# RaffaeleGalliera/melissa

Hardware: AMD Instinct MI355X
Metric: env-steps/s (agent-decisions/s) L-DGN 50-node (higher is better)
Workload: dtype f32 (f32a)

## Files before the change

include/melissa_hip.h:

```cpp
#ifndef MELISSA_HIP_H
#define MELISSA_HIP_H

#include <stddef.h>
#include <stdint.h>

#ifdef __cplusplus
extern "C" {
#endif

typedef int32_t mel_status;
#define MEL_OK                 0
#define MEL_ERR_INVALID_ARG   -1
#define MEL_ERR_SHAPE         -2
#define MEL_ERR_UNSUPPORTED   -3
#define MEL_ERR_WORKSPACE     -4
#define MEL_ERR_LAUNCH        -5

#define MEL_MAX_NODES        128
#define MEL_SET_WORDS(n)     (((n) + 63) / 64)
#define MEL_NODE_COLS          8
#define MEL_MAX_HEAD_LAYERS    6

#define MEL_MODEL_LDGN         0
#define MEL_MODEL_HLDGN        1
// ... 30 lines not shown
    int32_t n_layers;
} mel_mlp;

typedef struct mel_weights {
    int32_t model;
    int32_t in_dim;
    int32_t n_actions;
    int32_t dueling;
    mel_mlp   encoder;
    mel_gatv2 conv1;
    mel_gatv2 conv2;
    mel_mlp   q_head;
    mel_mlp   v_head;
    int32_t precision;
    int32_t flags;
    const void* prepared;
    const void* tables;
    int32_t tables_nodes;
    int32_t reserved;
} mel_weights;
#define MEL_FWD_PLAN_READY 1
#define MEL_FWD_INTEGER_FEATURES 2

#define MEL_PREC_F32  0
#define MEL_PREC_BF16 1
#define MEL_PREC_F32_SPLIT 2
#define MEL_PREC_F32_AUTO 3

size_t mel_prepared_weights_bytes(const mel_weights* w);
mel_status mel_prepare_weights(const mel_weights* w, void* prepared, size_t bytes, void* stream);

size_t mel_feature_tables_bytes(const mel_weights* w, int32_t n_nodes);
mel_status mel_prepare_feature_tables(const mel_weights* w, int32_t n_nodes, void* tables, size_t bytes, void* stream);

size_t mel_workspace_bytes(const mel_weights* w, int64_t bs, int32_t n_nodes);

mel_status mel_ldgn_forward(const mel_weights* w, const float* obs, int64_t bs, int32_t n_nodes,
                            int32_t obs_width, float* logits, void* workspace, size_t ws_bytes,
                            void* stream);

typedef struct mel_select {
    int32_t*        act;
    float           eps;
    uint32_t        seed;
    const uint32_t* step_dev;
    const uint64_t* live;
    int32_t         n_nodes;
    int32_t         reserved;
    const float*    eps_dev;
} mel_select;

size_t mel_workspace_bytes_agents(const mel_weights* w, int64_t bs, int32_t n_nodes, int64_t rows_cap);
mel_status mel_plan_pointers(const mel_weights* w, int64_t bs, int32_t n_nodes, int64_t rows_cap, void* workspace,
                             void** out5);
mel_status mel_ldgn_forward_agents(const mel_weights* w, const float* obs, int64_t bs, int32_t n_nodes,
                                   int32_t obs_stride, const uint64_t* agent_mask, int64_t rows_cap,
                                   float* logits, int32_t* row_offsets, const mel_select* select,
                                   void* workspace, size_t ws_bytes, void* stream);

mel_status mel_dgnr_forward(const mel_weights* w, const float* obs, int64_t bs, int32_t n_nodes,
                            int32_t obs_width, float* logits, void* workspace, size_t ws_bytes,
                            void* stream);
mel_status mel_dgnr_forward_agents(const mel_weights* w, const float* obs, int64_t bs, int32_t n_nodes,
                                   int32_t obs_stride, const uint64_t* agent_mask, int64_t rows_cap,
                                   float* logits, int32_t* row_offsets, const mel_select* select,
                                   void* workspace, size_t ws_bytes, void* stream);
// ... 346 lines not shown
```

melissa_amd/_lib.py:

```python
from __future__ import annotations

import ctypes as C
import os

from . import build as _build

MAX_HEAD_LAYERS = 6
TD_GROUP_ROWS, TD_MAX_BATCH, TD_MAX_ACTIONS = 64, 65536, 8
MAX_NODES = 128


def set_words(n: int) -> int:
    return (int(n) + 63) // 64


def check_n_nodes(n: int, what: str):
    if not (1 <= int(n) <= MAX_NODES):
        raise ValueError(f"{what}: {n} nodes per graph is outside [1, {MAX_NODES}] - the MI355X kernels hold one graph per "
                         f"wavefront (at most two nodes per lane, node sets of at most two 64-bit words)")
MODEL_LDGN, MODEL_HLDGN, MODEL_DGNR = 0, 1, 2
CONV_GATV2, CONV_TRANSFORMER = 0, 1
AGG = {"max": 0, "mean": 1, "add": 2}
OK, ERR_INVALID_ARG, ERR_SHAPE, ERR_UNSUPPORTED, ERR_WORKSPACE, ERR_LAUNCH = 0, -1, -2, -3, -4, -5
ENV_SCALARS, ENV_LOGGER_STATS = 16, 10
S_ORIGIN, S_SELECTION, S_SKIP, S_NUM_MOVES, S_WORLD_MSGS, S_NEW_ROUND, S_EPISODE, S_MOVE_CURSOR, \
    S_DECISIONS, S_DONE_COUNT, S_EPISODES_DONE, S_ERROR, S_EP_CURSOR = range(13)
SET_HAS_MESSAGE, SET_ORIGIN, SET_INTERESTED, SET_SCRIPTED, SET_TRUNCATED, SET_ALIVE, SET_TERMINATED, \
    SET_AGENTS = range(8)

EXPORTS = ("mel_wait_counter", "mel_feature_tables_bytes", "mel_prepare_feature_tables", "mel_prepared_weights_bytes", "mel_prepare_weights", "mel_transpose_f32", "mel_episode_refill", "mel_episode_test_seeds", "mel_abi_sizeof", "mel_radius_graph", "mel_gat_forward", "mel_gat_backward", "mel_pool_forward", "mel_pool_backward",
           "mel_gemm_bf16", "mel_convert_bf16", "mel_hldgn_forward_envs", "mel_hldgn_forward_envs_select", "mel_plan_pointers", "mel_select_action_envs", "mel_dgnr_forward", "mel_dgnr_forward_agents", "mel_gemm_f32", "mel_gemm_f32_t", "mel_gemm_f32_splitk", "mel_gemm_f32_split", "mel_replay_sample", "mel_replay_sample_prio", "mel_replay_update_priority", "mel_adam_step", "mel_workspace_bytes", "mel_workspace_bytes_agents", "mel_ldgn_forward_agents",
           "mel_select_action_rows", "mel_ldgn_forward", "mel_hldgn_forward", "mel_forward_tap",
           "mel_select_action", "mel_env_state_bytes", "mel_env_bind", "mel_env_reset", "mel_env_step",
           "mel_env_observe", "mel_env_round", "mel_prof_create", "mel_prof_destroy", "mel_prof_attach", "mel_prof_reset",
           "mel_prof_read", "mel_last_error", "mel_version", "mel_mpr_sets", "mel_exploration_schedule", "mel_td_target", "mel_td_loss")
PREC_F32, PREC_BF16, PREC_F32_SPLIT, PREC_F32_AUTO = 0, 1, 2, 3
FWD_PLAN_READY = 1
FWD_INTEGER_FEATURES = 2
HEURISTICS = {None: 0, "simple_broadcast": 1, "broadcast_if_any_interested": 2, "silent": 3, "mpr": 4}
LOGGER_KEYS = ("total_messages_transmitted", "coverage", "messages_sent", "messages_received", "n_neighbours",
               "interested_agents", "coverage_interested_fraction", "coverage_interested_count",
               "uninterested_with_message", "episode_rewards_sum")
N_STAGES = 14
STAGE_NAMES = ("plan", "encoder", "conv1_lin", "conv1_lin_r", "conv1_att", "conv2_lin", "conv2_lin_r", "conv2_att",
               "head_hidden", "head_tail", "select", "env_step", "env_reset", "env_observe")


class MelLinear(C.Structure):
    _fields_ = [("weight", C.c_void_p), ("bias", C.c_void_p), ("in_dim", C.c_int32), ("out_dim", C.c_int32)]


class MelGatv2(C.Structure):
    _fields_ = [("lin_l", MelLinear), ("lin_r", MelLinear), ("att", C.c_void_p), ("bias", C.c_void_p),
                ("heads", C.c_int32), ("channels", C.c_int32), ("lin_v", MelLinear), ("kind", C.c_int32),
                ("reserved", C.c_int32)]


class MelMlp(C.Structure):
    _fields_ = [("layer", MelLinear * MAX_HEAD_LAYERS), ("n_layers", C.c_int32)]


class MelWeights(C.Structure):
    _fields_ = [("model", C.c_int32), ("in_dim", C.c_int32), ("n_actions", C.c_int32), ("dueling", C.c_int32),
# ... 163 lines not shown
    lib.mel_select_action.argtypes = [vp, vp, i64, i32, C.c_float, vp, vp, vp, vp, vp]
    lib.mel_env_state_bytes.restype = sz
    lib.mel_env_state_bytes.argtypes = [i32, i32]
    lib.mel_env_bind.restype = i32
    lib.mel_env_bind.argtypes = [E, i32, i32, vp]
    lib.mel_env_reset.restype = i32
    lib.mel_env_reset.argtypes = [E, P, vp, vp, i64, i32, O, vp]
    lib.mel_env_step.restype = i32
    lib.mel_env_step.argtypes = [E, P, vp, vp, i64, O, vp, i32, vp]
    lib.mel_env_round.restype = i32
    lib.mel_env_round.argtypes = [E, P, vp, vp, vp, vp, i32, i32, vp, C.POINTER(MelRoundReplay), vp]
    lib.mel_adam_step.restype = i32
    lib.mel_adam_step.argtypes = [C.POINTER(MelAdamTensors), C.c_float, C.c_float, C.c_float, C.c_float, C.c_float, C.c_double, vp]
    lib.mel_td_target.restype = i32
    lib.mel_td_target.argtypes = [vp, vp, vp, vp, i64, i32, vp, vp]
    lib.mel_td_loss.restype = i32
    lib.mel_td_loss.argtypes = [vp, vp, vp, vp, vp, i64, i32, i32, i32, vp, vp, vp, vp, sz, vp]
    lib.mel_replay_sample.restype = i32
    lib.mel_replay_sample.argtypes = [C.POINTER(MelRoundReplay), i64, i32, i32, i32, C.POINTER(C.c_float), C.c_uint64, vp, vp,
                                      C.POINTER(MelReplayBatch), vp]
    lib.mel_replay_sample_prio.restype = i32
    lib.mel_replay_sample_prio.argtypes = [C.POINTER(MelRoundReplay), C.POINTER(MelReplayPriority), i64, i32, i32, i32,
                                           C.POINTER(C.c_float), C.c_uint64, vp, C.POINTER(MelReplayBatch), vp, vp]
    lib.mel_replay_update_priority.restype = i32
    lib.mel_replay_update_priority.argtypes = [C.POINTER(MelReplayPriority), i64, i32, i32, i32, vp, vp, vp, vp, vp]
    lib.mel_env_observe.restype = i32
    lib.mel_env_observe.argtypes = [E, vp, i64, O, vp]
    lib.mel_mpr_sets.restype = i32
    lib.mel_mpr_sets.argtypes = [vp, i32, i32, vp, vp]
    lib.mel_feature_tables_bytes.restype = sz
    lib.mel_feature_tables_bytes.argtypes = [W, i32]
    lib.mel_prepare_feature_tables.restype = i32
    lib.mel_prepare_feature_tables.argtypes = [W, i32, vp, sz, vp]
    lib.mel_prepared_weights_bytes.restype = sz
    lib.mel_prepared_weights_bytes.argtypes = [W]
    lib.mel_prepare_weights.restype = i32
    lib.mel_prepare_weights.argtypes = [W, vp, sz, vp]
    lib.mel_transpose_f32.restype = i32
    lib.mel_transpose_f32.argtypes = [vp, i32, i64, i32, vp, i32, vp]
    lib.mel_gemm_f32.restype = i32
    lib.mel_gemm_f32.argtypes = [vp, i32, vp, vp, vp, i32, i64, i32, i32, i32, i32, vp]
    lib.mel_wait_counter.restype = i32
    lib.mel_wait_counter.argtypes = [vp, C.c_uint32, C.c_uint32, vp]
    lib.mel_episode_test_seeds.restype = i32
    lib.mel_episode_test_seeds.argtypes = [vp, i32, vp]
    lib.mel_episode_refill.restype = i32
    lib.mel_episode_refill.argtypes = [C.POINTER(MelEpisodeStream), C.POINTER(MelGraphPool), P, E, i32, i32, vp]
    lib.mel_prof_create.restype = vp
    lib.mel_prof_create.argtypes = [i32]
    lib.mel_prof_destroy.restype = None
    lib.mel_prof_destroy.argtypes = [vp]
    lib.mel_prof_attach.restype = None
    lib.mel_prof_attach.argtypes = [vp]
    lib.mel_prof_reset.restype = None
    lib.mel_prof_reset.argtypes = [vp]
    lib.mel_prof_read.restype = i32
    lib.mel_prof_read.argtypes = [vp, C.POINTER(C.c_double), C.POINTER(C.c_int64)]
    _lib = lib
    return lib


def last_error() -> str:
    return load().mel_last_error().decode()


def check(status: int, what: str = ""):
# ... 12 lines not shown
```

melissa_amd/build.py:

```python
from __future__ import annotations

import hashlib
import os
import subprocess
import sys

HERE = os.path.dirname(os.path.abspath(__file__))
CSRC = os.path.join(HERE, "csrc")
LIB_DIR = os.path.join(HERE, "lib")
LIB_PATH = os.path.join(LIB_DIR, "libmelissa_hip.so")
SOURCES = ["fwd.hip", "env.hip", "grad.hip"]
HEADERS = ["common.hpp", "gemm_f32.hpp", "gemm_walk.hpp", "gemm_bf16.hpp", "gemm_split.hpp", "gemm_ring.hpp", "gemm_launch.hpp", "plan.hpp", "plan_masks.hpp", "attention.hpp", "heads.hpp", "episode_stream.hpp", "replay_prio.hpp", "td.hpp", os.path.join("..", "..", "include", "melissa_hip.h")]


def _hipcc() -> str:
    for cand in (os.environ.get("HIPCC"), "/opt/rocm/bin/hipcc"):
        if cand and os.path.exists(cand):
            return cand
    return "hipcc"


HASH_PATH = LIB_PATH + ".srchash"


def source_hash() -> str:
    h = hashlib.sha256()
    h.update(os.environ.get("MEL_HIPCC_FLAGS", "").encode())
    for rel in SOURCES + HEADERS:
        path = os.path.join(CSRC, rel)
        if os.path.exists(path):
            h.update(rel.encode())
            h.update(open(path, "rb").read())
    return h.hexdigest()


def is_stale() -> bool:
    if not os.path.exists(LIB_PATH) or not os.path.exists(HASH_PATH):
        return True
    return open(HASH_PATH).read().strip() != source_hash()


def build_library(force: bool = False, verbose: bool = False) -> str:
    srcs = [os.path.join(CSRC, s) for s in SOURCES if os.path.exists(os.path.join(CSRC, s))]
    if not force and not is_stale():
        return LIB_PATH
# ... 22 lines not shown
```

melissa_amd/csrc/fwd.hip:

```cpp
#include <cmath>

#include "common.hpp"
#include "gemm_launch.hpp"
#include "plan.hpp"
#include "attention.hpp"
#include "heads.hpp"

namespace mel {

static thread_local char g_err[512] = "";
void set_error(const char* fmt, ...) {
    va_list ap;
    va_start(ap, fmt);
    vsnprintf(g_err, sizeof(g_err), fmt, ap);
    va_end(ap);
}

static thread_local Profiler* g_prof = nullptr;
Profiler* current_profiler() { return g_prof; }

template <int W>
__global__ __launch_bounds__(256, 2) void plan_enc_kernel(PlanListsArgs pa, GemmBatch batch, int gemm_blocks) {
    if ((int)blockIdx.x < gemm_blocks) gemm_f32_tile<2, 2, 1, 1, GEMM_MODE_ENC>(batch, (int)blockIdx.x);
    else plan_lists_body<W>(pa, (int)blockIdx.x - gemm_blocks);
}

__global__ __launch_bounds__(256, 2) void fid_enc_kernel(const float* __restrict__ obs, int bs, int n, int obs_stride, int node_cols,
                                                         PlanBuffers p, int table_rows, GemmBatch batch, int gemm_blocks) {
    if ((int)blockIdx.x < gemm_blocks) gemm_f32_tile<2, 2, 1, 1, GEMM_MODE_ENC>(batch, (int)blockIdx.x);
    else feature_ids_body(obs, bs, n, obs_stride, node_cols, p, table_rows, (int)blockIdx.x - gemm_blocks);
}

struct Dims {
    int64_t bs;
    int n;
    int64_t rows_cap;
    int64_t u1_cap;
    int64_t u2_cap;
};

static Dims make_dims(int64_t bs, int n, int64_t rows_cap, bool single_agent) {
    Dims d;
    d.bs = bs, d.n = n, d.rows_cap = rows_cap;
    d.u1_cap = single_agent ? bs * (n < 34 ? n : 34) : bs * n;
    d.u2_cap = bs * n;
    return d;
}

struct FwdLayout {
    PlanBuffers plan;
    float* h0;
    float* xl1;
    float* xr1;
    float* h1;
    float* xl2;
    float* xr2;
    float* xcat;
// ... 341 lines not shown
        }
        const bool out16 = bf && !(i + 2 == nl);
        in_q = out, ld_q = ld_v = ldo;
        in_v = out16 ? reinterpret_cast<const float*>(reinterpret_cast<const uint16_t*>(out) + q.out_dim) : out + q.out_dim;
    }
    if (bf && nl < 2) return fail(MEL_ERR_UNSUPPORTED, "bf16 path needs at least one hidden layer in the heads");
    const mel_linear& ql = w->q_head.layer[nl - 1];
    const mel_linear& vl = w->v_head.layer[nl - 1];
    StageScope t(MEL_STAGE_HEAD_TAIL, s);
    MEL_LAUNCH(dueling_tail_kernel, dim3((rows + 3) / 4), dim3(256), 0, s, in_q, ld_q, ql.in_dim, in_v, ld_v,
                       vl.in_dim, ql, vl, (int)rows, rows_dev, w->dueling, logits, select ? *select : mel_select{});
    return check_launch("dueling tail");
}

struct FeatureTables {
    float* h0;
    float* xl;
    float* xr;
};
static size_t table_elem_bytes(const mel_weights* w) { return w->precision == MEL_PREC_BF16 ? 2 : 4; }
static FeatureTables carve_tables(const mel_weights* w, int n, void* buf, size_t* bytes) {
    const size_t T = (size_t)n * FEATURE_TUPLES_PER_DEGREE, es = table_elem_bytes(w);
    const int hidden = w->encoder.layer[1].out_dim, hc = w->conv1.heads * w->conv1.channels;
    const bool hl = w->model == MEL_MODEL_HLDGN;
    const int srcw = hl ? 2 * hc : (w->conv1.kind == MEL_CONV_TRANSFORMER ? 2 * hc : hc);
    Carver c(buf);
    FeatureTables t;
    t.h0 = reinterpret_cast<float*>(c.take<char>(T * hidden * es));
    t.xl = reinterpret_cast<float*>(c.take<char>(T * srcw * es));
    t.xr = hl ? nullptr : reinterpret_cast<float*>(c.take<char>(T * hc * es));
    if (bytes) *bytes = c.off;
    return t;
}
static mel_status run_feature_tables(const mel_weights* w, const ProjWeights& pw, int n, const FeatureTables& t, hipStream_t s,
                                     bool encoder_done = false) {
    const int T = n * FEATURE_TUPLES_PER_DEGREE;
    const int hidden = w->encoder.layer[1].out_dim, hc = w->conv1.heads * w->conv1.channels;
    const int bf = w->precision == MEL_PREC_BF16, sp = w->precision == MEL_PREC_F32_SPLIT;
    const bool tconv = w->conv1.kind == MEL_CONV_TRANSFORMER, hl = w->model == MEL_MODEL_HLDGN;
    if (!encoder_done) {
        GemmArgs g;
        g.feat_domain = 1, g.in_dim = w->in_dim, g.enc_w = w->encoder.layer[0].weight, g.enc_b = w->encoder.layer[0].bias;
        g.W = pw.enc1, g.bias = w->encoder.layer[1].bias, g.bf16 = bf, g.split = sp;
        if (bf) g.W = w->encoder.layer[1].weight, g.bf16 = 0, g.y_bf16 = 1;
        g.Y = t.h0, g.ldy = hidden, g.M = T, g.N = hidden, g.K = w->encoder.layer[0].out_dim, g.relu = 1;
        StageScope sc(MEL_STAGE_ENCODER, s);
        if (mel_status st = launch_gemm(g, GEMM_MODE_ENC, s, "encoder (feature tuples)", T)) return st;
    }
    StageScope sc(MEL_STAGE_CONV1_LIN, s);
    if (hl) {
        GemmArgs g;
        g.A = t.h0, g.lda = hidden, g.W = pw.c1l, g.W_hi = pw.c1r, g.bf16 = bf, g.split = sp;
        g.bias = w->conv1.lin_l.bias, g.bias_hi = w->conv1.lin_r.bias, g.split_n = hc;
        g.Y = t.xl, g.ldy = 2 * hc, g.M = T, g.N = 2 * hc, g.K = hidden;
        return launch_gemm(g, GEMM_MODE_PLAIN, s, "conv1.lin_l|lin_r (feature tuples)");
    }
    const int srcw = tconv ? 2 * hc : hc;
    GemmArgs g[2];
    g[0].bf16 = g[1].bf16 = bf, g[0].split = g[1].split = sp;
    g[0].A = t.h0, g[0].lda = hidden, g[0].W = pw.c1l, g[0].bias = w->conv1.lin_l.bias;
    g[0].Y = t.xl, g[0].ldy = srcw, g[0].M = T, g[0].N = srcw, g[0].K = hidden;
    if (tconv) g[0].W_hi = pw.c1v, g[0].bias_hi = w->conv1.lin_v.bias, g[0].split_n = hc;
    g[1].A = t.h0, g[1].lda = hidden, g[1].W = pw.c1r, g[1].bias = w->conv1.lin_r.bias;
    g[1].Y = t.xr, g[1].ldy = hc, g[1].M = T, g[1].N = hc, g[1].K = hidden;
    const long hints[2] = {T, T};
    return launch_gemm_group(g, hints, 2, s, "conv1.lin_l + lin_r (feature tuples)", 1);
}

static mel_status ldgn_forward_impl(const mel_weights* w, const float* obs, const Dims& d, int obs_stride,
                                    const uint64_t* agent_mask, float* logits, int32_t* row_offsets_out,
                                    const mel_select* select, void* workspace, size_t ws_bytes, hipStream_t s) {
    if (!obs || !logits || !workspace) return fail(MEL_ERR_INVALID_ARG, "null obs/logits/workspace");
    const FwdLayout L = carve(w, d, workspace);
    if (ws_bytes < L.bytes) return fail(MEL_ERR_WORKSPACE, "workspace %zu < %zu bytes", ws_bytes, L.bytes);
    clear_stale_error();
    const int64_t bs = d.bs;
    const int n = d.n;
    const int node_cols = w->in_dim + 3;
    const int hidden = w->encoder.layer[1].out_dim, hc = w->conv1.heads * w->conv1.channels;
    const int latent = hidden + 2 * hc;
    const bool tconv = w->conv1.kind == MEL_CONV_TRANSFORMER;
    const int srcw = tconv ? 2 * hc : hc;
    const int R = (int)d.rows_cap, U1 = (int)d.u1_cap, U2 = (int)d.u2_cap;
    const int32_t* nL = L.plan.offL + bs;
    const int32_t* n1 = L.plan.off1 + bs;
    const int32_t* n2 = L.plan.off2 + bs;
    const bool single = agent_mask == nullptr;
    const int bf = w->precision == MEL_PREC_BF16;
    const int sp = w->precision == MEL_PREC_F32_SPLIT;
    ProjWeights pw, pw_alt;
    if (mel_status st = resolve_projections(w, L, pw, pw_alt, s)) return st;
    const long hintL = single ? bs : (n < 10 ? bs : bs * (long)(36 + n) / 18);
    const long hint1 = single ? bs * (long)(n < 8 ? n : 2 + n / 8) : (n < 10 ? bs * (long)n : bs * 2L * (18 + n) / 13);
    const long hint2 = single ? bs * (long)(n < 8 ? n : 1 + n / 4) : (n < 10 ? bs * (long)n : bs * 3L * (8 + n) / 11);
    const int T = n * FEATURE_TUPLES_PER_DEGREE;
    const bool table = (w->flags & MEL_FWD_INTEGER_FEATURES) && w->in_dim == 5 && hint1 + hint2 >= 2L * T;
    bool fused_enc = false;
    GemmArgs c2[2];
    c2[0].bf16 = c2[1].bf16 = bf, c2[0].split = c2[1].split = sp;
    c2[0].A = L.h1, c2[0].lda = hc;
    c2[0].W = pw.c2l, c2[0].bias = w->conv2.lin_l.bias;
    c2[0].Y = L.xl2, c2[0].ldy = srcw, c2[0].M = U1, c2[0].M_dev = n1, c2[0].N = srcw, c2[0].K = hc;
    if (tconv) c2[0].W_hi = pw.c2v, c2[0].bias_hi = w->conv2.lin_v.bias, c2[0].split_n = hc;
    c2[1].A = L.h1, c2[1].lda = hc, c2[1].arow = L.plan.arow_g;
    c2[1].W = pw.c2r, c2[1].bias = w->conv2.lin_r.bias;
    if (pw.alt) c2[0].Ws = pw.alt->c2l, c2[0].Ws_hi = tconv ? pw.alt->c2v : nullptr, c2[1].Ws = pw.alt->c2r;
    c2[1].Y = L.xr2, c2[1].ldy = hc, c2[1].M = R, c2[1].M_dev = nL, c2[1].N = hc, c2[1].K = hc;
    const long c2_hints[2] = {hint1, hintL};
    const ProjWeights* planes = sp ? &pw : pw.alt;
    GemmRequest c2_rq;
    c2_rq.group = true;
    PlaneBlocks c2_blocks[2];
    if (planes && hc % 4 == 0 && hc / 64 >= 4) {
        c2_blocks[0] = {planes->c2l_blk, tconv ? planes->c2v_blk : nullptr}, c2_blocks[1] = {planes->c2r_blk, nullptr};
        c2_rq.blocks = c2_blocks;
    }
    const GemmPlan conv2 = plan_gemm(c2, c2_hints, 2, c2_rq);

    {
        StageScope t(MEL_STAGE_PLAN, s);
        if (w->flags & MEL_FWD_PLAN_READY) {
            if (!agent_mask) return fail(MEL_ERR_INVALID_ARG, "MEL_FWD_PLAN_READY needs the agent-set entry points");
        } else {
            if (n > 64) MEL_LAUNCH(plan_masks_kernel<2>, dim3((bs + 3) / 4), dim3(256), 0, s, obs, (int)bs, n, obs_stride, node_cols, agent_mask, L.plan, 1);
            else MEL_LAUNCH(plan_masks_kernel<1>, dim3((bs + 3) / 4), dim3(256), 0, s, obs, (int)bs, n, obs_stride, node_cols, agent_mask, L.plan, 1);
            if (mel_status st = check_launch("plan_masks")) return st;
        }
        const int inline_scan = bs <= 8192;
        if (!inline_scan) {
            MEL_LAUNCH(plan_scan_kernel, dim3(1), dim3(1024), 0, s, (int)bs, L.plan);
            if (mel_status st = check_launch("plan_scan")) return st;
        }
        fused_enc = table && !sp && !(w->tables && w->tables_nodes == n);
        const PlanListsArgs pa{obs, (int)bs, n, obs_stride, node_cols, L.plan, row_offsets_out, tconv ? 0 : 1, inline_scan, table ? T : 0};
        if (fused_enc) {
            GemmArgs g;
            g.feat_domain = 1, g.in_dim = w->in_dim, g.enc_w = w->encoder.layer[0].weight, g.enc_b = w->encoder.layer[0].bias;
            g.W = bf ? w->encoder.layer[1].weight : pw.enc1, g.bias = w->encoder.layer[1].bias, g.y_bf16 = bf;
            g.Y = L.h0, g.ldy = hidden, g.M = T, g.N = hidden, g.K = w->encoder.layer[0].out_dim, g.relu = 1;
            GemmRequest rq;
            rq.mode = GEMM_MODE_ENC, rq.force_tile = MEL_TILE_64;
            const GemmPlan enc = plan_gemm(&g, nullptr, 1, rq);
            if (enc.status) return fail(enc.status, "encoder (feature tuples): %s", enc.why);
            const int tiles = enc.grid;
            if (n > 64) MEL_LAUNCH(plan_enc_kernel<2>, dim3(tiles + (int)((bs + 3) / 4)), dim3(256), 0, s, pa, enc.batch, tiles);
            else MEL_LAUNCH(plan_enc_kernel<1>, dim3(tiles + (int)((bs + 3) / 4)), dim3(256), 0, s, pa, enc.batch, tiles);
        } else if (n > 64) {
            MEL_LAUNCH(plan_lists_kernel<2>, dim3((bs + 3) / 4), dim3(256), 0, s, pa);
        } else {
            MEL_LAUNCH(plan_lists_kernel<1>, dim3((bs + 3) / 4), dim3(256), 0, s, pa);
        }
        if (mel_status st = check_launch("plan_lists")) return st;
    }
    {
        GemmArgs g;
        g.obs = obs, g.obs_width = obs_stride, g.n_nodes = n, g.in_dim = w->in_dim, g.node_cols = node_cols;
        g.nid = L.plan.nid2, g.enc_w = w->encoder.layer[0].weight, g.enc_b = w->encoder.layer[0].bias;
        g.W = pw.enc1, g.bias = w->encoder.layer[1].bias, g.bf16 = bf, g.split = sp;
        g.Y = L.h0, g.ldy = hidden, g.M = U2, g.M_dev = n2, g.N = hidden;
        g.K = w->encoder.layer[0].out_dim, g.relu = 1;
        StageScope t(MEL_STAGE_ENCODER, s);
        if (!table)
            if (mel_status st = launch_gemm(g, GEMM_MODE_ENC, s, "encoder", hint2)) return st;
    }
    FeatureTables ft{L.h0, L.xl1, L.xr1};
    if (table) {
        if (w->tables && w->tables_nodes == n) ft = carve_tables(w, n, const_cast<void*>(w->tables), nullptr);
        else if (mel_status st = run_feature_tables(w, pw, n, ft, s, fused_enc)) return st;
    }
    {
        GemmArgs g[2];
        g[0].bf16 = g[1].bf16 = bf, g[0].split = g[1].split = sp;
        g[0].A = L.h0, g[0].lda = hidden, g[0].W = pw.c1l, g[0].bias = w->conv1.lin_l.bias;
        g[0].Y = L.xl1, g[0].ldy = srcw, g[0].M = U2, g[0].M_dev = n2, g[0].N = srcw, g[0].K = hidden;
        if (tconv)
            g[0].W_hi = pw.c1v, g[0].bias_hi = w->conv1.lin_v.bias, g[0].split_n = hc;
        g[1].A = L.h0, g[1].lda = hidden, g[1].arow = L.plan.arow1;
        g[1].W = pw.c1r, g[1].bias = w->conv1.lin_r.bias;
        g[1].Y = L.xr1, g[1].ldy = hc, g[1].M = U1, g[1].M_dev = n1, g[1].N = hc, g[1].K = hidden;
        const long hints[2] = {hint2, hint1};
        StageScope t(MEL_STAGE_CONV1_LIN, s);
        if (!table)
            if (mel_status st = launch_gemm_group(g, hints, 2, s, "conv1.lin_l + lin_r", 1)) return st;
    }
    {
        AttArgs a{};
        a.xl = ft.xl, a.ld_l = srcw, a.xr = ft.xr, a.ld_r = hc, a.att = w->conv1.att, a.bias = w->conv1.bias;
        a.kind = w->conv1.kind, a.score_scale = 1.0f / sqrtf((float)w->conv1.channels), a.bf16 = bf;
        a.adj = L.plan.adj, a.bs = (int)bs, a.n = n;
        a.desc = L.plan.desc1, a.rows_dev = n1, a.rows_cap = U1, a.rows_hint = hint1;
        a.lanes_per_head = w->conv1.channels / (hc / 64);
        a.out = L.h1, a.ldo = hc, a.xcat = L.xcat, a.ld_cat = latent, a.hidden = hidden, a.h0 = ft.h0;
        if (conv2.kernel == GemmKernel::PLANES) a.out_planes = reinterpret_cast<uint16_t*>(L.h1);
        a.out_scale = L.plan.dm1;
        a.fid = table ? L.plan.fid : nullptr;
        StageScope t(MEL_STAGE_CONV1_ATT, s);
        if (mel_status st = launch_attend<ATT_ROWS>(a, hc, s, "conv1 attention")) return st;
    }
    {
        StageScope t(MEL_STAGE_CONV2_LIN, s);
// ... 14 lines not shown
}

}

using namespace mel;

extern "C" {

const char* mel_last_error(void) { return g_err; }
void mel_debug_fin_prof(unsigned long long* out5) {
#ifdef MEL_FIN_PROF
    (void)hipMemcpyFromSymbol(out5, HIP_SYMBOL(g_fin_prof), 5 * sizeof(unsigned long long));
    unsigned long long z[5] = {};
    (void)hipMemcpyToSymbol(HIP_SYMBOL(g_fin_prof), z, sizeof(z));
#else
    for (int i = 0; i < 5; ++i) out5[i] = 0;
#endif
}

#ifdef MEL_RING_PROF
void mel_debug_ring_prof(unsigned long long* out8) {
    (void)hipDeviceSynchronize();
    (void)hipMemcpyFromSymbol(out8, HIP_SYMBOL(g_ring_prof), 8 * sizeof(unsigned long long));
    unsigned long long z[8] = {0};
    (void)hipMemcpyToSymbol(HIP_SYMBOL(g_ring_prof), z, sizeof(z));
}
#endif
#ifdef MEL_GEMM_PROF
void mel_debug_gemm_prof(unsigned long long* out8) {
    (void)hipDeviceSynchronize();
    (void)hipMemcpyFromSymbol(out8, HIP_SYMBOL(g_gemm_prof), 8 * sizeof(unsigned long long));
    unsigned long long z[8] = {0};
    (void)hipMemcpyToSymbol(HIP_SYMBOL(g_gemm_prof), z, sizeof(z));
}
#endif
#ifdef MEL_SPLIT_PROF
void mel_debug_split_prof(unsigned long long* out16) {
    (void)hipDeviceSynchronize();
    (void)hipMemcpyFromSymbol(out16, HIP_SYMBOL(g_split_prof), 16 * sizeof(unsigned long long));
    unsigned long long z[16] = {0};
    (void)hipMemcpyToSymbol(HIP_SYMBOL(g_split_prof), z, sizeof(z));
}
#endif
#ifdef MEL_ATT_PROF
void mel_debug_att_prof(unsigned long long* out8) {
    (void)hipDeviceSynchronize();
    (void)hipMemcpyFromSymbol(out8, HIP_SYMBOL(g_att_prof), 8 * sizeof(unsigned long long));
    unsigned long long z[8] = {0};
    (void)hipMemcpyToSymbol(HIP_SYMBOL(g_att_prof), z, sizeof(z));
}
#endif
size_t mel_abi_sizeof(int32_t which) {
    switch (which) {
        case 0: return sizeof(mel_linear);
        case 1: return sizeof(mel_gatv2);
        case 2: return sizeof(mel_mlp);
        case 3: return sizeof(mel_weights);
        case 4: return sizeof(mel_select);
        case 5: return sizeof(mel_env_batch);
        case 6: return sizeof(mel_episode_pool);
        case 7: return sizeof(mel_env_obs);
        case 8: return sizeof(mel_round_replay);
        case 9: return sizeof(mel_graph_pool);
        case 10: return sizeof(mel_episode_stream);
        case 11: return sizeof(mel_replay_batch);
        case 12: return sizeof(mel_adam_tensors);
        case 13: return sizeof(mel_replay_priority);
        default: return 0;
    }
}
const char* mel_version(void) { return "melissa_hip 0.6 (gfx950)"; }

size_t mel_prepared_weights_bytes(const mel_weights* w) {
    if (!w || w->precision < MEL_PREC_F32 || w->precision > MEL_PREC_F32_AUTO) return 0;
    return prepared_elems(w) * sizeof(uint16_t);
}

size_t mel_feature_tables_bytes(const mel_weights* w, int32_t n_nodes) {
    if (!w || n_nodes < 1 || n_nodes > MEL_MAX_NODES || w->in_dim != 5 || w->encoder.n_layers != 2) return 0;
    size_t bytes = 0;
    (void)carve_tables(w, n_nodes, nullptr, &bytes);
    return bytes;
}

mel_status mel_prepare_feature_tables(const mel_weights* w, int32_t n_nodes, void* tables, size_t bytes, void* stream) {
    if (mel_status st = validate(w, w ? w->model : 0, 1, n_nodes, n_nodes * ((w ? w->in_dim : 5) + 3), false)) return st;
    if (w->in_dim != 5) return fail(MEL_ERR_UNSUPPORTED, "the node-feature table is defined for the 5 GraphEnv features");
    const size_t need = mel_feature_tables_bytes(w, n_nodes);
    if (!tables || bytes < need) return fail(MEL_ERR_WORKSPACE, "feature-table buffer %zu < %zu bytes", bytes, need);
    if (w->precision != MEL_PREC_F32 && !w->prepared)
        return fail(MEL_ERR_INVALID_ARG, "bf16 / split precision: prepare the weights first (mel_prepare_weights)");
    clear_stale_error();
    hipStream_t s = static_cast<hipStream_t>(stream);
    ProjWeights pw, pw_alt;
    FwdLayout none{};
    if (mel_status st = resolve_projections(w, none, pw, pw_alt, s)) return st;
    return run_feature_tables(w, pw, n_nodes, carve_tables(w, n_nodes, tables, nullptr), s);
}

mel_status mel_prepare_weights(const mel_weights* w, void* prepared, size_t bytes, void* stream) {
    if (!w) return fail(MEL_ERR_INVALID_ARG, "weights pointer is null");
    if (w->precision == MEL_PREC_F32) return MEL_OK;
    if (w->precision != MEL_PREC_BF16 && !has_planes(w)) return fail(MEL_ERR_INVALID_ARG, "precision=%d", w->precision);
    const size_t need = prepared_elems(w) * sizeof(uint16_t);
    if (!prepared || bytes < need) return fail(MEL_ERR_WORKSPACE, "prepared-weights buffer %zu < %zu bytes", bytes, need);
    clear_stale_error();
    ProjWeights pw, pw_alt;
    return resolve_projections(w, static_cast<uint16_t*>(prepared), pw, pw_alt, static_cast<hipStream_t>(stream), true);
}

size_t mel_workspace_bytes(const mel_weights* w, int64_t bs, int32_t n_nodes) {
    if (!w || bs <= 0 || n_nodes < 1 || n_nodes > MEL_MAX_NODES) return 0;
    return carve(w, make_dims(bs, n_nodes, bs, true), nullptr).bytes;
}

size_t mel_workspace_bytes_agents(const mel_weights* w, int64_t bs, int32_t n_nodes, int64_t rows_cap) {
    if (!w || bs <= 0 || n_nodes < 1 || n_nodes > MEL_MAX_NODES || rows_cap < 1) return 0;
    return carve(w, make_dims(bs, n_nodes, rows_cap, false), nullptr).bytes;
}

mel_status mel_ldgn_forward(const mel_weights* w, const float* obs, int64_t bs, int32_t n, int32_t obs_width,
                            float* logits, void* workspace, size_t ws_bytes, void* stream) {
    if (mel_status st = validate(w, MEL_MODEL_LDGN, bs, n, obs_width, true)) return st;
    return ldgn_forward_impl(w, obs, make_dims(bs, n, bs, true), obs_width, nullptr, logits, nullptr, nullptr,
                             workspace, ws_bytes, static_cast<hipStream_t>(stream));
}

mel_status mel_ldgn_forward_agents(const mel_weights* w, const float* obs, int64_t bs, int32_t n, int32_t obs_stride,
                                   const uint64_t* agent_mask, int64_t rows_cap, float* logits,
                                   int32_t* row_offsets, const mel_select* select, void* workspace,
// ... 418 lines not shown
```

melissa_amd/csrc/gemm_f32.hpp:

```cpp
#pragma once
#include "common.hpp"

namespace mel {

typedef float f32x16 __attribute__((ext_vector_type(16)));
typedef float f32x4 __attribute__((ext_vector_type(4)));

struct GemmArgs {
    const float* A = nullptr;
    int lda = 0;
    const int32_t* arow = nullptr;
    const float* rscale = nullptr;
    const float* obs = nullptr;
    int obs_width = 0, n_nodes = 0, in_dim = 0, node_cols = 0;
    const int32_t* nid = nullptr;
    int feat_domain = 0;
    const float* enc_w = nullptr;
    const float* enc_b = nullptr;
    const float* W = nullptr;
    const float* W_hi = nullptr;
    const float* bias = nullptr;
    const float* bias_hi = nullptr;
    int split_n = 0;
    float* Y = nullptr;
// ... 9 lines not shown
    const float* Ws = nullptr;
    const float* Ws_hi = nullptr;
    int ksplit = 0;
    long part_stride = 0;
};

constexpr int GEMM_MAX_GROUP = 4;
struct GemmBatch {
    GemmArgs p[GEMM_MAX_GROUP];
    int start[GEMM_MAX_GROUP + 1];
    int count;
};

}
#include "gemm_walk.hpp"
namespace mel {

constexpr int GEMM_BK = 32;
constexpr int GEMM_LDS_STRIDE = GEMM_BK + 4;

enum { GEMM_MODE_PLAIN = 0, GEMM_MODE_ENC = 1 };

template <class T>
__device__ __forceinline__ const T* weight_row(const GemmArgs& g, int n, size_t row_elems) {
    return (g.W_hi && n >= g.split_n) ? reinterpret_cast<const T*>(g.W_hi) + (size_t)(n - g.split_n) * row_elems
                                      : reinterpret_cast<const T*>(g.W) + (size_t)n * row_elems;
}

struct AChunk {
    const float* src;
    float x[8];
};

__device__ __forceinline__ void enc_features(const GemmArgs& g, int row, float x[8]) {
#pragma unroll
    for (int f = 0; f < 8; ++f) x[f] = 0.f;
    if (g.feat_domain) {
        const int deg = row / 40, rem = row - deg * 40;
        x[0] = (float)deg, x[1] = (float)(rem >> 3), x[2] = (float)((rem >> 2) & 1);
        x[3] = (float)((rem >> 1) & 1), x[4] = (float)(rem & 1);
        return;
    }
    const int id = g.nid ? g.nid[row] : row;
    const int b = id / g.n_nodes, node = id - b * g.n_nodes;
    const float* src = g.obs + (size_t)b * g.obs_width + node * g.node_cols + 2;
#pragma unroll
    for (int f = 0; f < 8; ++f)
        if (f < g.in_dim) x[f] = src[f];
}

template <int MODE>
__device__ __forceinline__ f32x4 fetch_a(const GemmArgs& g, const AChunk& c, int k0, int kc, const float* enc) {
    if constexpr (MODE == GEMM_MODE_PLAIN) {
        return *reinterpret_cast<const f32x4*>(c.src + k0);
    } else {
        float v[4];
#pragma unroll
        for (int e = 0; e < 4; ++e) {
            const float* wrow = enc + (k0 + kc + e) * 9;
            float s = wrow[8];
#pragma unroll
            for (int f = 0; f < 8; ++f) s = fmaf(wrow[f], c.x[f], s);
            v[e] = fmaxf(s, 0.f);
        }
        const f32x4 out = {v[0], v[1], v[2], v[3]};
        return out;
    }
}

struct EpilogueOperands {
    float bias;
    float sc[16];
};
__device__ __forceinline__ EpilogueOperands fetch_epilogue_operands(const GemmArgs& g, int m_lane, int n, int M) {
    EpilogueOperands o;
// ... 467 lines not shown
```

melissa_amd/csrc/gemm_launch.hpp:

```cpp
#pragma once
#include <cstdarg>
#include <cstdlib>
#include <type_traits>
#include "gemm_f32.hpp"
#include "gemm_bf16.hpp"
#include "gemm_split.hpp"
#include "gemm_ring.hpp"

namespace mel {

#ifndef MEL_PLANES_FROM
#define MEL_PLANES_FROM 129
#endif
#ifndef MEL_SPLIT_BIG_FROM
#define MEL_SPLIT_BIG_FROM 192
#endif

struct GemmTuning { bool no_planes; long planes_from; bool no_bf16_wide; };
static const GemmTuning& gemm_tuning() {
    static const GemmTuning t{getenv("MEL_NO_PLANES_GEMM") != nullptr,
                              getenv("MEL_PLANES_FROM") ? atol(getenv("MEL_PLANES_FROM")) : (long)MEL_PLANES_FROM,
                              getenv("MEL_NO_BF16_WIDE") != nullptr};
    return t;
}

enum class GemmKernel {
    NONE,
    F32,
    F32_PERSISTENT,
    RING,
    BF16,
    SPLIT,
    SPLIT_BIG,
    PLANES,
    BF16_WIDE,
};

struct GemmPlan {
    mel_status status = MEL_OK;
    char why[200] = "";
    GemmKernel kernel = GemmKernel::NONE;
    int mode = GEMM_MODE_PLAIN;
    int tm = 1, tn = 1;
    int ksplit = 1;
    GemmBatch batch{};
    int grid = 0, block = 0;

    GemmPlan& reject(mel_status code, const char* fmt, ...) __attribute__((format(printf, 3, 4))) {
        va_list ap;
        va_start(ap, fmt);
        vsnprintf(why, sizeof(why), fmt, ap);
        va_end(ap);
        kernel = GemmKernel::NONE, status = code;
        return *this;
    }
// ... 335 lines not shown
```

Baseline: 29.28 million.

## Fuse encoder and conv1 projections into one feature-table kernel

Adds a fused tile kernel that computes encoder layer 0, encoder layer 1 and the conv1 lin_l/lin_r projections for the integer-feature tuple table in a single pass. It keeps the intermediate hidden activations in LDS and stages weight slices through per-wave LDS using MFMA 32x32x2 f32. It is launched alongside the plan-lists kernel, replacing the separate encoder GEMM plus the run_feature_tables launches on the L-DGN f32 path. The intent is to remove extra kernel launches and global round-trips of h0. The cost is larger LDS use and register pressure, and encoder work is redone for each column group.

After: 30.28 million (median of 6 runs). +3.4%, better.

```diff
diff --git a/include/melissa_hip.h b/include/melissa_hip.h
--- a/include/melissa_hip.h
+++ b/include/melissa_hip.h
@@ -86,6 +86,7 @@
 
 size_t mel_feature_tables_bytes(const mel_weights* w, int32_t n_nodes);
 mel_status mel_prepare_feature_tables(const mel_weights* w, int32_t n_nodes, void* tables, size_t bytes, void* stream);
+mel_status mel_feature_tables_fused(const mel_weights* w, int32_t n_nodes, void* tables, size_t bytes, void* stream);
 
 size_t mel_workspace_bytes(const mel_weights* w, int64_t bs, int32_t n_nodes);
 
diff --git a/melissa_amd/_lib.py b/melissa_amd/_lib.py
--- a/melissa_amd/_lib.py
+++ b/melissa_amd/_lib.py
@@ -28,7 +28,7 @@
 SET_HAS_MESSAGE, SET_ORIGIN, SET_INTERESTED, SET_SCRIPTED, SET_TRUNCATED, SET_ALIVE, SET_TERMINATED, \
     SET_AGENTS = range(8)
 
-EXPORTS = ("mel_wait_counter", "mel_feature_tables_bytes", "mel_prepare_feature_tables", "mel_prepared_weights_bytes", "mel_prepare_weights", "mel_transpose_f32", "mel_episode_refill", "mel_episode_test_seeds", "mel_abi_sizeof", "mel_radius_graph", "mel_gat_forward", "mel_gat_backward", "mel_pool_forward", "mel_pool_backward",
+EXPORTS = ("mel_wait_counter", "mel_feature_tables_bytes", "mel_prepare_feature_tables", "mel_feature_tables_fused", "mel_prepared_weights_bytes", "mel_prepare_weights", "mel_transpose_f32", "mel_episode_refill", "mel_episode_test_seeds", "mel_abi_sizeof", "mel_radius_graph", "mel_gat_forward", "mel_gat_backward", "mel_pool_forward", "mel_pool_backward",
            "mel_gemm_bf16", "mel_convert_bf16", "mel_hldgn_forward_envs", "mel_hldgn_forward_envs_select", "mel_plan_pointers", "mel_select_action_envs", "mel_dgnr_forward", "mel_dgnr_forward_agents", "mel_gemm_f32", "mel_gemm_f32_t", "mel_gemm_f32_splitk", "mel_gemm_f32_split", "mel_replay_sample", "mel_replay_sample_prio", "mel_replay_update_priority", "mel_adam_step", "mel_workspace_bytes", "mel_workspace_bytes_agents", "mel_ldgn_forward_agents",
            "mel_select_action_rows", "mel_ldgn_forward", "mel_hldgn_forward", "mel_forward_tap",
            "mel_select_action", "mel_env_state_bytes", "mel_env_bind", "mel_env_reset", "mel_env_step",
@@ -258,6 +258,8 @@
     lib.mel_feature_tables_bytes.argtypes = [W, i32]
     lib.mel_prepare_feature_tables.restype = i32
     lib.mel_prepare_feature_tables.argtypes = [W, i32, vp, sz, vp]
+    lib.mel_feature_tables_fused.restype = i32
+    lib.mel_feature_tables_fused.argtypes = [W, i32, vp, sz, vp]
     lib.mel_prepared_weights_bytes.restype = sz
     lib.mel_prepared_weights_bytes.argtypes = [W]
     lib.mel_prepare_weights.restype = i32
diff --git a/melissa_amd/build.py b/melissa_amd/build.py
--- a/melissa_amd/build.py
+++ b/melissa_amd/build.py
@@ -10,7 +10,7 @@
 LIB_DIR = os.path.join(HERE, "lib")
 LIB_PATH = os.path.join(LIB_DIR, "libmelissa_hip.so")
 SOURCES = ["fwd.hip", "env.hip", "grad.hip"]
-HEADERS = ["common.hpp", "gemm_f32.hpp", "gemm_walk.hpp", "gemm_bf16.hpp", "gemm_split.hpp", "gemm_ring.hpp", "gemm_launch.hpp", "plan.hpp", "plan_masks.hpp", "attention.hpp", "heads.hpp", "episode_stream.hpp", "replay_prio.hpp", "td.hpp", os.path.join("..", "..", "include", "melissa_hip.h")]
+HEADERS = ["common.hpp", "gemm_f32.hpp", "gemm_walk.hpp", "gemm_bf16.hpp", "gemm_split.hpp", "gemm_ring.hpp", "gemm_table.hpp", "gemm_launch.hpp", "plan.hpp", "plan_masks.hpp", "attention.hpp", "heads.hpp", "episode_stream.hpp", "replay_prio.hpp", "td.hpp", os.path.join("..", "..", "include", "melissa_hip.h")]
 
 
 def _hipcc() -> str:
diff --git a/melissa_amd/csrc/fwd.hip b/melissa_amd/csrc/fwd.hip
--- a/melissa_amd/csrc/fwd.hip
+++ b/melissa_amd/csrc/fwd.hip
@@ -19,10 +19,17 @@
 static thread_local Profiler* g_prof = nullptr;
 Profiler* current_profiler() { return g_prof; }
 
-template <int W>
-__global__ __launch_bounds__(256, 2) void plan_enc_kernel(PlanListsArgs pa, GemmBatch batch, int gemm_blocks) {
-    if ((int)blockIdx.x < gemm_blocks) gemm_f32_tile<2, 2, 1, 1, GEMM_MODE_ENC>(batch, (int)blockIdx.x);
-    else plan_lists_body<W>(pa, (int)blockIdx.x - gemm_blocks);
+template <int W, bool FUSED = false>
+__global__ __launch_bounds__(256, 2) void plan_enc_kernel(PlanListsArgs pa, std::conditional_t<FUSED, TableArgs, GemmBatch> work,
+                                                          int gemm_blocks) {
+    if constexpr (FUSED) {
+        __shared__ __attribute__((aligned(16))) float lds[TBL_LDS_FLOATS];
+        if ((int)blockIdx.x < gemm_blocks) table_fused_tile(work, (int)blockIdx.x, lds);
+        else plan_lists_body<W>(pa, (int)blockIdx.x - gemm_blocks);
+    } else {
+        if ((int)blockIdx.x < gemm_blocks) gemm_f32_tile<2, 2, 1, 1, GEMM_MODE_ENC>(work, (int)blockIdx.x);
+        else plan_lists_body<W>(pa, (int)blockIdx.x - gemm_blocks);
+    }
 }
 
 __global__ __launch_bounds__(256, 2) void fid_enc_kernel(const float* __restrict__ obs, int bs, int n, int obs_stride, int node_cols,
@@ -430,6 +437,25 @@
     if (bytes) *bytes = c.off;
     return t;
 }
+static bool table_fuses(const mel_weights* w) {
+    const int hc = w->conv1.heads * w->conv1.channels, K0 = w->encoder.layer[0].out_dim;
+    return w->model == MEL_MODEL_LDGN && w->conv1.kind != MEL_CONV_TRANSFORMER &&
+           (w->precision == MEL_PREC_F32 || w->precision == MEL_PREC_F32_AUTO) && w->in_dim == 5 && w->encoder.n_layers == 2 &&
+           K0 == TBL_HIDDEN && w->encoder.layer[1].out_dim == TBL_HIDDEN &&
+           w->conv1.lin_l.in_dim == TBL_HIDDEN && hc % 32 == 0 && (2 * hc) % TBL_BN == 0;
+}
+static TableArgs fused_table_args(const mel_weights* w, const ProjWeights& pw, int n, const FeatureTables& t) {
+    const int hc = w->conv1.heads * w->conv1.channels;
+    TableArgs a;
+    a.T = n * FEATURE_TUPLES_PER_DEGREE, a.in_dim = w->in_dim;
+    a.enc_w = w->encoder.layer[0].weight, a.enc_b = w->encoder.layer[0].bias;
+    a.W1 = pw.enc1, a.b1 = w->encoder.layer[1].bias;
+    a.Wl = pw.c1l, a.Wr = pw.c1r, a.bl = w->conv1.lin_l.bias, a.br = w->conv1.lin_r.bias;
+    a.split_n = hc, a.N = 2 * hc;
+    a.h0 = t.h0, a.xl = t.xl, a.xr = t.xr;
+    return a;
+}
+
 static mel_status run_feature_tables(const mel_weights* w, const ProjWeights& pw, int n, const FeatureTables& t, hipStream_t s,
                                      bool encoder_done = false) {
     const int T = n * FEATURE_TUPLES_PER_DEGREE;
@@ -493,7 +519,7 @@
     const long hint2 = single ? bs * (long)(n < 8 ? n : 1 + n / 4) : (n < 10 ? bs * (long)n : bs * 3L * (8 + n) / 11);
     const int T = n * FEATURE_TUPLES_PER_DEGREE;
     const bool table = (w->flags & MEL_FWD_INTEGER_FEATURES) && w->in_dim == 5 && hint1 + hint2 >= 2L * T;
-    bool fused_enc = false;
+    bool fused_enc = false, fused_table = false;
     GemmArgs c2[2];
     c2[0].bf16 = c2[1].bf16 = bf, c2[0].split = c2[1].split = sp;
     c2[0].A = L.h1, c2[0].lda = hc;
@@ -530,8 +556,14 @@
             if (mel_status st = check_launch("plan_scan")) return st;
         }
         fused_enc = table && !sp && !(w->tables && w->tables_nodes == n);
+        fused_table = fused_enc && table_fuses(w) && !gemm_tuning().no_fused_table;
         const PlanListsArgs pa{obs, (int)bs, n, obs_stride, node_cols, L.plan, row_offsets_out, tconv ? 0 : 1, inline_scan, table ? T : 0};
-        if (fused_enc) {
+        if (fused_table) {
+            const TableArgs ta = fused_table_args(w, pw, n, FeatureTables{L.h0, L.xl1, L.xr1});
+            const int tiles = table_items(ta);
+            if (n > 64) MEL_LAUNCH((plan_enc_kernel<2, true>), dim3(tiles + (int)((bs + 3) / 4)), dim3(256), 0, s, pa, ta, tiles);
+            else MEL_LAUNCH((plan_enc_kernel<1, true>), dim3(tiles + (int)((bs + 3) / 4)), dim3(256), 0, s, pa, ta, tiles);
+        } else if (fused_enc) {
             GemmArgs g;
             g.feat_domain = 1, g.in_dim = w->in_dim, g.enc_w = w->encoder.layer[0].weight, g.enc_b = w->encoder.layer[0].bias;
             g.W = bf ? w->encoder.layer[1].weight : pw.enc1, g.bias = w->encoder.layer[1].bias, g.y_bf16 = bf;
@@ -564,6 +596,7 @@
     FeatureTables ft{L.h0, L.xl1, L.xr1};
     if (table) {
         if (w->tables && w->tables_nodes == n) ft = carve_tables(w, n, const_cast<void*>(w->tables), nullptr);
+        else if (fused_table) {}
         else if (mel_status st = run_feature_tables(w, pw, n, ft, s, fused_enc)) return st;
     }
     {
@@ -644,6 +677,14 @@
     (void)hipMemcpyFromSymbol(out8, HIP_SYMBOL(g_gemm_prof), 8 * sizeof(unsigned long long));
     unsigned long long z[8] = {0};
     (void)hipMemcpyToSymbol(HIP_SYMBOL(g_gemm_prof), z, sizeof(z));
+}
+#endif
+#ifdef MEL_TABLE_PROF
+void mel_debug_table_prof(unsigned long long* out8) {
+    (void)hipDeviceSynchronize();
+    (void)hipMemcpyFromSymbol(out8, HIP_SYMBOL(g_table_prof), 8 * sizeof(unsigned long long));
+    unsigned long long z[8] = {0};
+    (void)hipMemcpyToSymbol(HIP_SYMBOL(g_table_prof), z, sizeof(z));
 }
 #endif
 #ifdef MEL_SPLIT_PROF
@@ -708,6 +749,23 @@
     FwdLayout none{};
     if (mel_status st = resolve_projections(w, none, pw, pw_alt, s)) return st;
     return run_feature_tables(w, pw, n_nodes, carve_tables(w, n_nodes, tables, nullptr), s);
+}
+
+mel_status mel_feature_tables_fused(const mel_weights* w, int32_t n_nodes, void* tables, size_t bytes, void* stream) {
+    if (mel_status st = validate(w, w ? w->model : 0, 1, n_nodes, n_nodes * ((w ? w->in_dim : 5) + 3), false)) return st;
+    if (!table_fuses(w)) return fail(MEL_ERR_UNSUPPORTED, "the one-launch table is built for GATv2 L-DGN at f32 / f32-auto precision, hidden = %d", TBL_HIDDEN);
+    const size_t need = mel_feature_tables_bytes(w, n_nodes);
+    if (!tables || bytes < need) return fail(MEL_ERR_WORKSPACE, "feature-table buffer %zu < %zu bytes", bytes, need);
+    if (w->precision != MEL_PREC_F32 && !w->prepared)
+        return fail(MEL_ERR_INVALID_ARG, "bf16 / split precision: prepare the weights first (mel_prepare_weights)");
+    clear_stale_error();
+    hipStream_t s = static_cast<hipStream_t>(stream);
+    ProjWeights pw, pw_alt;
+    FwdLayout none{};
+    if (mel_status st = resolve_projections(w, none, pw, pw_alt, s)) return st;
+    const TableArgs ta = fused_table_args(w, pw, n_nodes, carve_tables(w, n_nodes, tables, nullptr));
+    MEL_LAUNCH(table_fused_kernel, dim3(table_items(ta)), dim3(256), 0, s, ta);
+    return check_launch("feature tables, one launch");
 }
 
 mel_status mel_prepare_weights(const mel_weights* w, void* prepared, size_t bytes, void* stream) {
diff --git a/melissa_amd/csrc/gemm_f32.hpp b/melissa_amd/csrc/gemm_f32.hpp
--- a/melissa_amd/csrc/gemm_f32.hpp
+++ b/melissa_amd/csrc/gemm_f32.hpp
@@ -65,15 +65,17 @@
     float x[8];
 };
 
+__device__ __forceinline__ void tuple_features(int row, float x[8]) {
+#pragma unroll
+    for (int f = 0; f < 8; ++f) x[f] = 0.f;
+    const int deg = row / 40, rem = row - deg * 40;
+    x[0] = (float)deg, x[1] = (float)(rem >> 3), x[2] = (float)((rem >> 2) & 1);
+    x[3] = (float)((rem >> 1) & 1), x[4] = (float)(rem & 1);
+}
 __device__ __forceinline__ void enc_features(const GemmArgs& g, int row, float x[8]) {
+    if (g.feat_domain) return tuple_features(row, x);
 #pragma unroll
     for (int f = 0; f < 8; ++f) x[f] = 0.f;
-    if (g.feat_domain) {
-        const int deg = row / 40, rem = row - deg * 40;
-        x[0] = (float)deg, x[1] = (float)(rem >> 3), x[2] = (float)((rem >> 2) & 1);
-        x[3] = (float)((rem >> 1) & 1), x[4] = (float)(rem & 1);
-        return;
-    }
     const int id = g.nid ? g.nid[row] : row;
     const int b = id / g.n_nodes, node = id - b * g.n_nodes;
     const float* src = g.obs + (size_t)b * g.obs_width + node * g.node_cols + 2;
diff --git a/melissa_amd/csrc/gemm_launch.hpp b/melissa_amd/csrc/gemm_launch.hpp
--- a/melissa_amd/csrc/gemm_launch.hpp
+++ b/melissa_amd/csrc/gemm_launch.hpp
@@ -6,6 +6,7 @@
 #include "gemm_bf16.hpp"
 #include "gemm_split.hpp"
 #include "gemm_ring.hpp"
+#include "gemm_table.hpp"
 
 namespace mel {
 
@@ -16,11 +17,11 @@
 #define MEL_SPLIT_BIG_FROM 192
 #endif
 
-struct GemmTuning { bool no_planes; long planes_from; bool no_bf16_wide; };
+struct GemmTuning { bool no_planes; long planes_from; bool no_bf16_wide; bool no_fused_table; };
 static const GemmTuning& gemm_tuning() {
     static const GemmTuning t{getenv("MEL_NO_PLANES_GEMM") != nullptr,
                               getenv("MEL_PLANES_FROM") ? atol(getenv("MEL_PLANES_FROM")) : (long)MEL_PLANES_FROM,
-                              getenv("MEL_NO_BF16_WIDE") != nullptr};
+                              getenv("MEL_NO_BF16_WIDE") != nullptr, getenv("MEL_NO_FUSED_TABLE") != nullptr};
     return t;
 }
 
diff --git a/melissa_amd/csrc/gemm_table.hpp b/melissa_amd/csrc/gemm_table.hpp
--- /dev/null
+++ b/melissa_amd/csrc/gemm_table.hpp
@@ -0,0 +1,217 @@
+#pragma once
+#include "gemm_f32.hpp"
+
+namespace mel {
+
+constexpr int TBL_BM = 32, TBL_BN = 256;
+constexpr int TBL_HIDDEN = 128;
+constexpr int TBL_A_STRIDE = TBL_HIDDEN + 4;
+constexpr int TBL_LDS_FLOATS = TBL_BM * TBL_A_STRIDE + TBL_HIDDEN * 9 + 4 * 64 * GEMM_LDS_STRIDE;
+
+struct TableArgs {
+    int T = 0;
+    int in_dim = 0;
+    const float* enc_w = nullptr;
+    const float* enc_b = nullptr;
+    const float* W1 = nullptr;
+    const float* b1 = nullptr;
+    const float* Wl = nullptr;
+    const float* Wr = nullptr;
+    const float* bl = nullptr;
+    const float* br = nullptr;
+    int split_n = 0, N = 0;
+    float* h0 = nullptr;
+    float* xl = nullptr;
+    float* xr = nullptr;
+};
+
+static inline int table_items(const TableArgs& a) { return ((a.T + TBL_BM - 1) / TBL_BM) * (a.N / TBL_BN); }
+
+#ifdef MEL_TABLE_PROF
+__device__ unsigned long long g_table_prof[8];
+#define TBL_T() __builtin_readcyclecounter()
+#define TBL_STAMP(i) do { const unsigned long long t_ = TBL_T(); tp[i] = t_ - tl; tl = t_; } while (0)
+#else
+#define TBL_STAMP(i)
+#endif
+
+__device__ __forceinline__ void table_stage_handoff() {
+    __builtin_amdgcn_fence(__ATOMIC_RELEASE, "wavefront");
+    __builtin_amdgcn_wave_barrier();
+    __builtin_amdgcn_fence(__ATOMIC_ACQUIRE, "wavefront");
+}
+
+__device__ __forceinline__ void table_fused_tile(const TableArgs& a, const int block, float* lds) {
+    const int ncg = a.N / TBL_BN;
+    const int m0 = (block / ncg) * TBL_BM, cg = block % ncg;
+    const int T = a.T;
+    const int tid = threadIdx.x, lane = tid & 63, wid = tid >> 6;
+    const int r = lane & 31, h = lane >> 5;
+#ifdef MEL_TABLE_PROF
+    unsigned long long tp[5], tl = TBL_T();
+    const unsigned long long t00 = tl;
+#endif
+    float* ablk = lds;
+    float* enc = lds + TBL_BM * TBL_A_STRIDE;
+
+    float e0[5];
+#pragma unroll
+    for (int u = 0; u < 5; ++u) {
+        const int i = tid + 256 * u, k = i / 9, f = i - k * 9;
+        e0[u] = 0.f;
+        if (i < TBL_HIDDEN * 9) e0[u] = f == 8 ? a.enc_b[k] : (f < a.in_dim ? a.enc_w[(size_t)k * a.in_dim + f] : 0.f);
+    }
+    const float bias1 = a.b1 ? a.b1[wid * 32 + r] : 0.f;
+    float biasc[2];
+#pragma unroll
+    for (int j = 0; j < 2; ++j) {
+        const int n = cg * TBL_BN + wid * 64 + j * 32 + r;
+        const float* bp = n >= a.split_n ? a.br : a.bl;
+        biasc[j] = bp ? bp[n >= a.split_n ? n - a.split_n : n] : 0.f;
+    }
+    const int lrow = lane >> 3, lk = (lane & 7) * 4;
+    float* wp = enc + TBL_HIDDEN * 9 + wid * 64 * GEMM_LDS_STRIDE;
+    f32x4 w1r[4][4], wcr[4][8];
+    {
+        const float* src = a.W1 + (size_t)(wid * 32 + lrow) * TBL_HIDDEN + lk;
+#pragma unroll
+        for (int sg = 0; sg < 4; ++sg)
+#pragma unroll
+            for (int g = 0; g < 4; ++g) w1r[sg][g] = *reinterpret_cast<const f32x4*>(src + (size_t)8 * g * TBL_HIDDEN + 32 * sg);
+    }
+    const float* wc_src[8];
+#pragma unroll
+    for (int g = 0; g < 8; ++g) {
+        const int n = cg * TBL_BN + wid * 64 + 8 * g + lrow;
+        wc_src[g] = (n >= a.split_n ? a.Wr + (size_t)(n - a.split_n) * TBL_HIDDEN : a.Wl + (size_t)n * TBL_HIDDEN) + lk;
+    }
+#pragma unroll
+    for (int sg = 0; sg < 2; ++sg)
+#pragma unroll
+        for (int g = 0; g < 8; ++g) wcr[sg][g] = *reinterpret_cast<const f32x4*>(wc_src[g] + 32 * sg);
+
+#pragma unroll
+    for (int u = 0; u < 5; ++u)
+        if (tid + 256 * u < TBL_HIDDEN * 9) enc[tid + 256 * u] = e0[u];
+    __syncthreads();
+    {
+        const int row = tid >> 3, kc = (tid & 7) * 4;
+        float x[8];
+        tuple_features(min(m0 + row, T - 1), x);
+#pragma unroll
+        for (int k0 = 0; k0 < TBL_HIDDEN; k0 += 32) {
+            float v[4];
+#pragma unroll
+            for (int e = 0; e < 4; ++e) {
+                const float* w = enc + (k0 + kc + e) * 9;
+                float s = w[8];
+#pragma unroll
+                for (int f = 0; f < 8; ++f) s = fmaf(w[f], x[f], s);
+                v[e] = fmaxf(s, 0.f);
+            }
+            const f32x4 out = {v[0], v[1], v[2], v[3]};
+            *reinterpret_cast<f32x4*>(ablk + row * TBL_A_STRIDE + k0 + kc) = out;
+        }
+    }
+    __syncthreads();
+    TBL_STAMP(0);
+
+    const float* afrag = ablk + r * TBL_A_STRIDE + 4 * h;
+    f32x16 acc1;
+#pragma unroll
+    for (int e = 0; e < 16; ++e) acc1[e] = 0.f;
+    const float* wfrag = wp + r * GEMM_LDS_STRIDE + 4 * h;
+    float* wslot = wp + lrow * GEMM_LDS_STRIDE + lk;
+#pragma unroll
+    for (int sg = 0; sg < 4; ++sg) {
+#pragma unroll
+        for (int g = 0; g < 4; ++g) *reinterpret_cast<f32x4*>(wslot + 8 * g * GEMM_LDS_STRIDE) = w1r[sg][g];
+        table_stage_handoff();
+#pragma unroll
+        for (int q = 0; q < 4; ++q) {
+            const f32x4 av = *reinterpret_cast<const f32x4*>(afrag + 32 * sg + 8 * q);
+            const f32x4 bv = *reinterpret_cast<const f32x4*>(wfrag + 8 * q);
+#pragma unroll
+            for (int kk = 0; kk < 4; ++kk) acc1 = __builtin_amdgcn_mfma_f32_32x32x2f32(av[kk], bv[kk], acc1, 0, 0, 0);
+        }
+        table_stage_handoff();
+    }
+#pragma unroll
+    for (int sg = 2; sg < 4; ++sg)
+#pragma unroll
+        for (int g = 0; g < 8; ++g) wcr[sg][g] = *reinterpret_cast<const f32x4*>(wc_src[g] + 32 * sg);
+    TBL_STAMP(1);
+    __syncthreads();
+    {
+        const int n = wid * 32 + r;
+        const float bias = bias1;
+        float v[16];
+#pragma unroll
+        for (int e = 0; e < 16; ++e) v[e] = fmaxf(acc1[e] + bias, 0.f);
+#pragma unroll
+        for (int e = 0; e < 16; ++e) ablk[(4 * h + (e & 3) + 8 * (e >> 2)) * TBL_A_STRIDE + n] = v[e];
+        if (cg == 0) {
+            float* col = a.h0 + n;
+#pragma unroll
+            for (int e = 0; e < 16; ++e) {
+                const int m = m0 + 4 * h + (e & 3) + 8 * (e >> 2);
+                if (m < T) col[(size_t)m * TBL_HIDDEN] = v[e];
+            }
+        }
+    }
+    __syncthreads();
+    TBL_STAMP(2);
+
+    f32x16 acc[2];
+#pragma unroll
+    for (int j = 0; j < 2; ++j)
+#pragma unroll
+        for (int e = 0; e < 16; ++e) acc[j][e] = 0.f;
+#pragma unroll
+    for (int sg = 0; sg < 4; ++sg) {
+#pragma unroll
+        for (int g = 0; g < 8; ++g) *reinterpret_cast<f32x4*>(wslot + 8 * g * GEMM_LDS_STRIDE) = wcr[sg][g];
+        table_stage_handoff();
+#pragma unroll
+        for (int q = 0; q < 4; ++q) {
+            const f32x4 av = *reinterpret_cast<const f32x4*>(afrag + 32 * sg + 8 * q);
+            f32x4 bv[2];
+#pragma unroll
+            for (int j = 0; j < 2; ++j) bv[j] = *reinterpret_cast<const f32x4*>(wfrag + j * 32 * GEMM_LDS_STRIDE + 8 * q);
+#pragma unroll
+            for (int kk = 0; kk < 4; ++kk)
+#pragma unroll
+                for (int j = 0; j < 2; ++j) acc[j] = __builtin_amdgcn_mfma_f32_32x32x2f32(av[kk], bv[j][kk], acc[j], 0, 0, 0);
+        }
+        table_stage_handoff();
+    }
+    TBL_STAMP(3);
+#pragma unroll
+    for (int j = 0; j < 2; ++j) {
+        const int n = cg * TBL_BN + wid * 64 + j * 32 + r;
+        const bool hi = n >= a.split_n;
+        const int c = hi ? n - a.split_n : n, ldy = hi ? a.N - a.split_n : a.split_n;
+        const float bias = biasc[j];
+        float* col = (hi ? a.xr : a.xl) + c;
+#pragma unroll
+        for (int e = 0; e < 16; ++e) {
+            const int m = m0 + 4 * h + (e & 3) + 8 * (e >> 2);
+            if (m < T) col[(size_t)m * ldy] = acc[j][e] + bias;
+        }
+    }
+#ifdef MEL_TABLE_PROF
+    asm volatile("s_waitcnt vmcnt(0)" ::: "memory");
+    TBL_STAMP(4);
+    if (tid == 0) {
+        for (int i = 0; i < 5; ++i) atomicAdd(&g_table_prof[i], tp[i]);
+        atomicAdd(&g_table_prof[5], TBL_T() - t00), atomicAdd(&g_table_prof[6], 1ull);
+    }
+#endif
+}
+
+__global__ __launch_bounds__(256, 2) void table_fused_kernel(TableArgs a) {
+    __shared__ __attribute__((aligned(16))) float lds[TBL_LDS_FLOATS];
+    table_fused_tile(a, (int)blockIdx.x, lds);
+}
+
+}
```
